# kerrm/vlite-fast

Measured on AMD Instinct MI355X. Metric: Msamp/s/antenna (dual-pol) and x real-time @128 MS/s; % HBM roofline, higher is better.
Workload: dtype f32

## Files before the change

### include/pb_hip.h

```cpp
#ifndef PB_HIP_H
#define PB_HIP_H

#include <stddef.h>
#include <stdint.h>

#ifdef __cplusplus
extern "C" {
#endif

#define PB_NFFT 12500
#define PB_NCHAN 6251
#define PB_NSCRUNCH 8
#define PB_NKURTO 500
#define PB_CHANMIN 2155
#define PB_CHANMAX 6250
#define PB_NCHANOUT 4096
#define PB_BLK_PER_FFT 25
#define PB_VDIF_FRAME 5032
#define PB_VDIF_DATA 5000
#define PB_FRAMES_PER_SEC 25600

#define PB_OK 0
#define PB_EINVAL (-22)
#define PB_ENOMEM (-12)
// ... 72 lines not shown
                         size_t nsamp_per_pol);
int pb_submit_vdif(pb_handle *h, int ant, int seg0, const uint8_t *block, size_t nbytes);
int pb_submit_vdif_at(pb_handle *h, int ant, int seg0, const uint8_t *block, size_t nbytes,
                      int64_t second, int64_t frame0);
int pb_input_dev(pb_handle *h, int ant, void **dptr, size_t *nbytes);

int pb_process(pb_handle *h, int nseg, int inject_now);

int pb_set_frb_params(pb_handle *h, float dm, float width_rows, float amp);

int pb_fetch(pb_handle *h, int ant, int seg0, int nseg, uint8_t *raw_codes, uint8_t *kur_codes,
             float *weights, float *ave_raw, float *ave_kur);
int pb_select_set(pb_handle *h, int set);
int pb_fetch_ptr(pb_handle *h, int ant, int stream, const uint8_t **codes);
int pb_output_dev(pb_handle *h, int ant, int stream, void **codes, void **ave);

int pb_coadd_local(pb_handle *h, int nseg, float *d_sum, int accumulate);
int pb_coadd_local_codes(pb_handle *h, int nseg, float *d_sum, int accumulate);
#define PB_COADD_MAX_LEAVES 32
int pb_coadd_tree_order(int n, int32_t *order);
int pb_coadd_local_tree(pb_handle *h, int nseg, const int32_t *ant_order, int n, float *d_dst);
int pb_coadd_tree(pb_handle *h, const float *const *d_leaves, int n, float *d_dst, size_t nfloat);
int pb_coadd_digitise(pb_handle *h, const float *d_sum, size_t nfloat, int nant_total, uint8_t *d_codes);
int pb_coadd_publish(pb_handle *h, const uint8_t *d_codes, size_t nbytes);
int pb_set_coadd_target(pb_handle *h, float *d_sum);
int pb_coadd_release(pb_handle *h);
int pb_set_coadd_stream(pb_handle *h, void *stream);
int pb_coadd_finish(pb_handle *h, int nseg, const float *d_sum, int nant_total,
                    uint8_t *codes_host);
int pb_coadd_fetch_ptr(pb_handle *h, int age, const uint8_t **codes);

int pb_profile(pb_handle *h, int enable);
int pb_get_timers(pb_handle *h, pb_timers *out, int reset);
int pb_debug_fetch(pb_handle *h, int what, int ant, int seg, void *dst, size_t nbytes);

int pb_debug_dag_check(pb_handle *h, float kur_lo, float kur_hi, uint64_t *nchecked, uint64_t *nmismatch,
                       float *bands4);

int pb_channelize_f32(pb_handle *h, const float *x, int nrows, int taps, float *out);

typedef struct pb_search pb_search;
int pb_search_create(int device, int nchan, int max_samples, float fch1_mhz, float foff_mhz, float tsamp_s,
                     float dm_min, float dm_max, float dm_step, int boxcar_max, const int *zap_ranges,
                     int nzap, pb_search **out);
int pb_search_create_list(int device, int nchan, int max_samples, float fch1_mhz, float foff_mhz, float tsamp_s,
                          const float *dm_list, int ndm, int boxcar_max, const int *zap_ranges, int nzap,
                          pb_search **out);
void pb_search_destroy(pb_search *s);
const char *pb_search_last_error(const pb_search *s);
int pb_search_info(const pb_search *s, int *ndm, int *nbox, int *max_delay);
int pb_search_run(pb_search *s, const void *codes, int codes_on_device, int nsamp, int nbit, float *snr,
                  uint8_t *width_log2, uint32_t *series, float *stats, int *tout);
int pb_search_set_baseline(pb_search *s, int window_samples);
int pb_search_peaks(pb_search *s, const void *codes, int codes_on_device, int nsamp, int nbit, float threshold,
                    int32_t *peaks, int max_out, int *npeaks, int *tout);
int pb_search_timers(const pb_search *s, float *ms6);

int pb_search_set_rfi(pb_search *s, int narrow, int broad, float tol, int rfi_boxcar_max);
int pb_search_rfi_info(const pb_search *s, uint64_t *n_narrow, int *n_broad_samples, float *ms);
int pb_search_fetch_clean(pb_search *s, uint8_t *xt, size_t nbytes);

int pb_search_set_cutouts(pb_search *s, int nsub, int nt, int ndmrow, int max_cands);
int pb_search_cutouts(pb_search *s, const int32_t *cands3, int n, uint32_t *ft, uint32_t *ft_hits, uint32_t *dt,
                      uint32_t *dt_hits);
int pb_search_cutout_timers(const pb_search *s, float *ms2);

int pb_search_set_refine(pb_search *s, int nstep, int half_window, int wmax, int max_cands);
int pb_search_refine(pb_search *s, const int32_t *req_i2, const float *req_f2, int n, int32_t *status, double *sn_dm,
                     int32_t *kbest, double *opt_sn, int32_t *opt_loc, uint32_t *series);
int pb_search_refine_timers(const pb_search *s, float *ms2);

int pb_search_set_pol(pb_search *s, int off_len, int guard, int nrm, double rm_lo, double rm_step, int max_cands);
int pb_search_pol(pb_search *s, const int32_t *req3, int n, int32_t *on, int32_t *non, int32_t *off, int32_t *noff, double *F,
                  int32_t *kbest, double *summary);
int pb_search_pol_cutouts(pb_search *s, const int32_t *cands3, int n, uint32_t *pft, uint32_t *pft_hits);
int pb_search_pol_fetch(pb_search *s, int which, uint8_t *out, size_t nbytes);
int pb_search_pol_timers(const pb_search *s, float *ms3);

#define PB_GIANT_WORDS 8
int pb_search_set_giants(pb_search *s, int sep_time, int sep_dm, int sep_filter, int max_giants);
int pb_search_giants(pb_search *s, float thresh, int t_lo, int t_hi, int32_t *cands, int max_out, int *ncands, int *ngiants,
                     int *overflow);
int pb_search_giant_list(pb_search *s, int32_t *out, int max_out, int *n);
int pb_search_set_planes(pb_search *s, const float *snr, const uint8_t *width_log2, int tout);
int pb_search_giant_timers(const pb_search *s, float *ms3, int *nsweeps);

int pb_search_set_gulp(pb_search *s, int keep_max);
int pb_search_push_f32(pb_search *s, const float *plane, int plane_on_device, int nsamp, float scale, int *fill);
int pb_search_push(pb_search *s, const void *codes, int codes_on_device, int nsamp, int nbit, int *fill);
int pb_search_gulp_peaks(pb_search *s, float threshold, int32_t *peaks, int max_out, int *npeaks, int *tout);
int pb_search_gulp_run(pb_search *s, float *snr, uint8_t *width_log2, uint32_t *series, float *stats, int *tout);
int pb_search_gulp_advance(pb_search *s, int keep);
int pb_search_gulp_fetch(pb_search *s, uint8_t *xt, size_t nbytes, int *fill);
int pb_search_gulp_timers(const pb_search *s, float *ms3);

void *pb_host_alloc(size_t nbytes);
void pb_host_free(void *p);

const char *pb_version(void);

#ifdef __cplusplus
}
#endif
#endif
```

### vlite-fast_amd/csrc/search_internal.h

```cpp
#pragma once
#include <hip/hip_runtime.h>

#include <cmath>
#include <cstdint>
#include <cstring>
#include <initializer_list>
#include <string>
#include <vector>

#include "pb_hip.h"

#define SEARCH_LOCAL __attribute__((visibility("hidden")))

struct pb_search {
    int device = 0, nchan = 0, max_samples = 0, ndm = 0, nbox = 0;
    float fch1 = 0.f, foff = 0.f, tsamp = 0.f;
    double dm_last = 0, ftop = 0;
    int max_delay = 0;
    uint8_t *d_codes = nullptr, *d_xt = nullptr;
    int32_t *d_delay = nullptr;
    int32_t *d_chans = nullptr;
    int nact = 0;
    uint32_t *d_D = nullptr;
    float *d_stats = nullptr;
    float *d_snr = nullptr;
    uint8_t *d_wid = nullptr;
    uint64_t *d_P = nullptr;
    int32_t *d_peaks = nullptr;
    int max_peaks = 1 << 20;
    int baseline = 0;
    int last_tout = 0, last_nsamp = 0;
    int plane_tout = 0;
    float ms[6] = {};
    hipEvent_t ev[7] = {};
    size_t tpitch = 0;
    hipStream_t stream = nullptr;
    std::string err;
    size_t ppitch() const { return tpitch + 8; }

    struct {
        int narrow = 0, broad = 0, nbox = 5;
        float tol = 5.0f;
        int ran = 0;
        int32_t *d_zdelay = nullptr;
        uint8_t *d_med = nullptr;
        uint32_t *d_z = nullptr;
        uint64_t *d_zP = nullptr;
        float *d_zstats = nullptr, *d_zsnr = nullptr;
        uint8_t *d_zwid = nullptr;
        int32_t *d_tlist = nullptr;
        unsigned long long *d_rcnt = nullptr;
        hipEvent_t ev[1] = {};
        uint64_t n_narrow = 0;
        int n_broad = 0;
        float ms = 0.f;
    } rfi;
    struct {
        int nsub = 0, nt = 0, ndmrow = 0, max = 0;
        int32_t *d_req = nullptr;
        int32_t *d_sub = nullptr;
        uint32_t *d_out = nullptr;
        uint32_t *h_out = nullptr;
        hipEvent_t ev[3] = {};
        float ms[2] = {};
    } cut;
    struct {
        int nstep = 0, H = 0, wmax = 0, max = 0;
        double *d_g = nullptr;
        int32_t *d_reqi = nullptr;
        float *d_reqf = nullptr;
        int32_t *d_out = nullptr;
        int32_t *h_out = nullptr;
        hipEvent_t ev[3] = {};
        float ms[2] = {};
    } rf;
    struct {
        int sep_time = 0, sep_dm = 0, sep_filter = 0, max = 0;
        int last = 0;
        int sweeps = 0;
        int32_t *d_cnt = nullptr, *d_row = nullptr;
        int32_t *d_giants = nullptr;
        int32_t *d_lab = nullptr;
        unsigned long long *d_best = nullptr;
        int32_t *d_acc = nullptr;
        int32_t *d_tile = nullptr;
        int32_t *d_out = nullptr;
        int32_t *h_out = nullptr;
        hipEvent_t ev[4] = {};
        float ms[3] = {};
    } gi;
    struct {
        int keep_max = 0;
// ... 32 lines not shown
extern SEARCH_LOCAL std::string g_search_err;

static inline int search_fail(pb_search *s, const char *fn, const std::string &what)
{
    (s ? s->err : g_search_err) = std::string(fn) + ": " + what;
    return PB_EINVAL;
}

#define SCHK(s, call)                                                         \
    do {                                                                      \
        hipError_t e_ = (call);                                               \
        if (e_ != hipSuccess) {                                               \
            (s)->err = std::string(#call) + ": " + hipGetErrorString(e_);     \
            return PB_EHIP;                                                   \
        }                                                                     \
    } while (0)

static inline int search_enter(pb_search *s, const char *fn, bool on, const char *off_msg, bool ready, const char *idle_msg)
{
    if (!s) return search_fail(nullptr, fn, "no search handle");
    if (!on) return search_fail(s, fn, off_msg);
    if (!ready) return search_fail(s, fn, idle_msg);
    return PB_OK;
}

static inline float search_ms(hipEvent_t a, hipEvent_t b)
{
    float ms = 0.f;
    return hipEventElapsedTime(&ms, a, b) == hipSuccess ? ms : 0.f;
}

static inline int search_get_ms(const pb_search *s, const float *ms, int n, float *out)
{
    if (!s || !out) return PB_EINVAL;
    for (int i = 0; i < n; ++i) out[i] = ms[i];
    return PB_OK;
}

static inline void search_release(std::initializer_list<void *> dev, void *host, hipEvent_t *ev, int nev)
{
    for (void *p : dev)
        if (p) (void)hipFree(p);
    if (host) (void)hipHostFree(host);
    for (int i = 0; i < nev; ++i)
        if (ev[i]) (void)hipEventDestroy(ev[i]);
}

SEARCH_LOCAL void search_rfi_free(pb_search *s);
SEARCH_LOCAL void search_cutouts_free(pb_search *s);
SEARCH_LOCAL void search_refine_free(pb_search *s);
SEARCH_LOCAL void search_giants_free(pb_search *s);
SEARCH_LOCAL void search_gulp_free(pb_search *s);
SEARCH_LOCAL void search_pol_free(pb_search *s);

SEARCH_LOCAL int search_pol_transpose(pb_search *s, const uint8_t *codes, int nsamp);
SEARCH_LOCAL void search_cutout_ft_launch(pb_search *s, const uint8_t *plane, int n, uint32_t *ft, uint32_t *fth);

SEARCH_LOCAL int search_block(pb_search *s, int nsamp, float thresh, bool want_peaks, bool cleaned);
SEARCH_LOCAL int search_run_out(pb_search *s, float *snr, uint8_t *width_log2, uint32_t *series, float *stats, int *tout_out);
SEARCH_LOCAL int search_peaks_out(pb_search *s, int32_t *peaks, int max_out, int *npeaks, int *tout_out);
```

### vlite-fast_amd/csrc/search_run.hip

```cpp
#include "search_internal.h"
#include "search_dev.h"

std::string g_search_err;

__global__ __launch_bounds__(256) void k_transpose_codes(const uint8_t *__restrict__ codes, uint8_t *__restrict__ xt,
                                                         int T, int nchan, int nbit, size_t tpitch)
{
    __shared__ uint8_t tile[64][65];
    const int t0 = blockIdx.x * 64, c0 = blockIdx.y * 64;
    const int per = 8 / nbit, maskv = (1 << nbit) - 1;
    for (int i = threadIdx.x; i < 64 * 64; i += 256) {
        const int tt = i / 64, cc = i % 64;
        const int t = t0 + tt, c = c0 + cc;
        uint8_t v = 0;
        if (t < T && c < nchan) {
            const size_t n = (size_t)t * nchan + c;
            v = (codes[n / per] >> (nbit * (n % per))) & maskv;
        }
        tile[tt][cc] = v;
    }
    __syncthreads();
    for (int i = threadIdx.x; i < 64 * 64; i += 256) {
        const int cc = i / 64, tt = i % 64;
        const int t = t0 + tt, c = c0 + cc;
// ... 410 lines not shown
    s->tsamp = tsamp_s;
    s->ndm = (int)dms.size();
    while ((1 << s->nbox) <= boxcar_max) s->nbox++;
    s->dm_last = dms.back();
    std::vector<int32_t> chans;
    for (int c = 0; c < nchan; ++c) {
        bool zap = false;
        for (int z = 0; z < nzap; ++z)
            if (c >= zap_ranges[2 * z] && c < zap_ranges[2 * z + 1]) zap = true;
        if (!zap) chans.push_back(c);
    }
    s->nact = (int)chans.size();
    if (s->nact == 0) {
        g_search_err = "pb_search_create: every channel is zapped";
        delete s;
        return PB_EINVAL;
    }
    std::vector<int32_t> delay((size_t)s->ndm * s->nact);
    const double ftop = foff_mhz < 0 ? fch1_mhz : fch1_mhz + (nchan - 1) * foff_mhz;
    s->ftop = ftop;
    int maxd = 0;
    for (int i = 0; i < s->ndm; ++i) {
        const double dm = dms[i];
        for (int k = 0; k < s->nact; ++k) {
            const double f = (double)fch1_mhz + (double)chans[k] * (double)foff_mhz;
            const int32_t di = delay_samples(dm, delay_chan_term(f, ftop), (double)tsamp_s);
            delay[(size_t)i * s->nact + k] = di;
            if (di > maxd) maxd = di;
        }
    }
    s->max_delay = maxd;
    s->tpitch = ((size_t)max_samples + 63) / 64 * 64;
    hipError_t e = hipSetDevice(device);
    if (e == hipSuccess) e = hipStreamCreateWithFlags(&s->stream, hipStreamNonBlocking);
    if (e == hipSuccess) e = hipMalloc((void **)&s->d_codes, (size_t)max_samples * nchan);
    if (e == hipSuccess) e = hipMalloc((void **)&s->d_xt, s->tpitch * nchan + 64);
    if (e == hipSuccess) e = hipMemset(s->d_xt, 0, s->tpitch * nchan + 64);
    if (e == hipSuccess) e = hipMalloc((void **)&s->d_delay, delay.size() * sizeof(int32_t));
    if (e == hipSuccess) e = hipMalloc((void **)&s->d_chans, chans.size() * sizeof(int32_t));
    if (e == hipSuccess) e = hipMemcpy(s->d_chans, chans.data(), chans.size() * sizeof(int32_t), hipMemcpyHostToDevice);
    if (e == hipSuccess) e = hipMalloc((void **)&s->d_D, (size_t)s->ndm * s->tpitch * sizeof(uint32_t));
    if (e == hipSuccess) e = hipMalloc((void **)&s->d_stats, (size_t)s->ndm * 2 * sizeof(float));
    if (e == hipSuccess) e = hipMalloc((void **)&s->d_snr, (size_t)s->ndm * s->tpitch * sizeof(float));
    if (e == hipSuccess) e = hipMalloc((void **)&s->d_wid, (size_t)s->ndm * s->tpitch);
    if (e == hipSuccess) e = hipMalloc((void **)&s->d_P, (size_t)s->ndm * s->ppitch() * sizeof(uint64_t));
    if (e == hipSuccess) e = hipMalloc((void **)&s->d_peaks, (size_t)(1 + 4 * s->max_peaks) * sizeof(int32_t));
    for (int i = 0; i < 7 && e == hipSuccess; ++i) e = hipEventCreate(&s->ev[i]);
    if (e == hipSuccess) e = hipMemcpy(s->d_delay, delay.data(), delay.size() * sizeof(int32_t), hipMemcpyHostToDevice);
    if (e != hipSuccess) {
        g_search_err = std::string("pb_search_create: ") + hipGetErrorString(e);
        pb_search_destroy(s);
        return PB_EHIP;
    }
    *out = s;
    return PB_OK;
}

void search_rfi_free(pb_search *s)
{
    search_release({s->rfi.d_zdelay, s->rfi.d_med, s->rfi.d_z, s->rfi.d_zP, s->rfi.d_zstats, s->rfi.d_zsnr, s->rfi.d_zwid,
                    s->rfi.d_tlist, s->rfi.d_rcnt}, nullptr, s->rfi.ev, 1);
    s->rfi = {};
}

extern "C" void pb_search_destroy(pb_search *s)
{
    if (!s) return;
    (void)hipSetDevice(s->device);
    if (s->stream) (void)hipStreamSynchronize(s->stream);
    search_rfi_free(s);
    search_cutouts_free(s);
    search_refine_free(s);
    search_giants_free(s);
    search_gulp_free(s);
    search_pol_free(s);
    search_release({s->d_codes, s->d_xt, s->d_delay, s->d_D, s->d_stats, s->d_snr, s->d_wid, s->d_P, s->d_peaks, s->d_chans},
                   nullptr, s->ev, 7);
    if (s->stream) (void)hipStreamDestroy(s->stream);
    delete s;
}

extern "C" int pb_search_info(const pb_search *s, int *ndm, int *nbox, int *max_delay)
{
    if (!s) return PB_EINVAL;
    if (ndm) *ndm = s->ndm;
    if (nbox) *nbox = s->nbox;
    if (max_delay) *max_delay = s->max_delay;
    return PB_OK;
}

extern "C" int pb_search_set_baseline(pb_search *s, int window_samples)
{
    if (!s || window_samples < 0) return PB_EINVAL;
    s->baseline = window_samples;
    return PB_OK;
}

extern "C" int pb_search_set_rfi(pb_search *s, int narrow, int broad, float tol, int rfi_boxcar_max)
{
    const char *fn = "pb_search_set_rfi";
    if (!(tol > 0) || !std::isfinite(tol)) return search_fail(s, fn, "tol must be > 0 and finite");
    if (rfi_boxcar_max < 1 || rfi_boxcar_max > 64 || (rfi_boxcar_max & (rfi_boxcar_max - 1)))
        return search_fail(s, fn, "rfi_boxcar_max must be a power of two in 1..64");
    if (!s) return search_fail(s, fn, "no search handle");
    if ((narrow || broad) && !s->rfi.d_rcnt) {
        const size_t tp = s->tpitch;
        SCHK(s, hipSetDevice(s->device));
        SCHK(s, hipMalloc((void **)&s->rfi.d_zdelay, (size_t)s->nact * sizeof(int32_t)));
        SCHK(s, hipMemset(s->rfi.d_zdelay, 0, (size_t)s->nact * sizeof(int32_t)));
        SCHK(s, hipMalloc((void **)&s->rfi.d_med, (size_t)s->nact));
        SCHK(s, hipMalloc((void **)&s->rfi.d_z, tp * sizeof(uint32_t)));
        SCHK(s, hipMalloc((void **)&s->rfi.d_zP, s->ppitch() * sizeof(uint64_t)));
        SCHK(s, hipMalloc((void **)&s->rfi.d_zstats, 2 * sizeof(float)));
        SCHK(s, hipMalloc((void **)&s->rfi.d_zsnr, tp * sizeof(float)));
        SCHK(s, hipMalloc((void **)&s->rfi.d_zwid, tp));
        SCHK(s, hipMalloc((void **)&s->rfi.d_tlist, tp * sizeof(int32_t)));
        SCHK(s, hipEventCreate(&s->rfi.ev[0]));
        SCHK(s, hipMalloc((void **)&s->rfi.d_rcnt, 2 * sizeof(unsigned long long)));
    }
    s->rfi.narrow = narrow != 0;
    s->rfi.broad = broad != 0;
    s->rfi.tol = tol;
    s->rfi.nbox = 0;
    while ((1 << s->rfi.nbox) <= rfi_boxcar_max) s->rfi.nbox++;
    return PB_OK;
}

static int search_clean(pb_search *s, int nsamp)
{
    const size_t ppitch = s->ppitch();
    SCHK(s, hipMemsetAsync(s->rfi.d_rcnt, 0, 2 * sizeof(unsigned long long), s->stream));
    k_rfi_narrow<<<s->nact, 256, 0, s->stream>>>(s->d_xt, s->d_chans, s->rfi.d_med, nsamp, s->tpitch, s->rfi.tol,
                                                 s->rfi.narrow, s->rfi.d_rcnt);
    if (s->rfi.broad) {
        dim3 gz((nsamp + DDM_TILE - 1) / DDM_TILE, 1);
        k_dedisperse<<<gz, 256, 0, s->stream>>>(s->d_xt, s->d_chans, s->rfi.d_zdelay, s->rfi.d_z, s->nact, 1, nsamp, s->tpitch,
                                                s->tpitch);
        k_prefix<<<1, 256, 0, s->stream>>>(s->rfi.d_z, s->rfi.d_zP, nsamp, s->tpitch, ppitch);
        k_series_stats<<<1, 256, 0, s->stream>>>(s->rfi.d_z, s->rfi.d_zP, s->rfi.d_zstats, nsamp, s->baseline, s->tpitch, ppitch);
        dim3 gb((nsamp + 255) / 256, 1);
        k_boxcar<<<gb, 256, 0, s->stream>>>(s->rfi.d_zP, s->rfi.d_zstats, s->rfi.d_zsnr, s->rfi.d_zwid, nsamp, s->rfi.nbox, s->baseline,
                                            s->tpitch, ppitch, 0.f, nullptr, 0);
        k_rfi_broad_list<<<gb, 256, 0, s->stream>>>(s->rfi.d_zsnr, s->rfi.d_zwid, nsamp, s->rfi.tol, 1 << (s->rfi.nbox - 1),
                                                    s->rfi.d_tlist, s->rfi.d_rcnt + 1);
        k_rfi_broad_mask<<<(s->nact + 3) / 4, 256, 0, s->stream>>>(s->d_xt, s->d_chans, s->rfi.d_med, s->rfi.d_tlist,
                                                                   s->rfi.d_rcnt + 1, s->nact, s->tpitch);
    }
    SCHK(s, hipEventRecord(s->rfi.ev[0], s->stream));
    return PB_OK;
}

int search_block(pb_search *s, int nsamp, float thresh, bool want_peaks, bool cleaned)
{
    const int tout = nsamp - s->max_delay;
    s->rfi.ran = s->rfi.narrow || s->rfi.broad;
    if (s->rfi.ran && cleaned) {
        SCHK(s, hipEventRecord(s->rfi.ev[0], s->stream));
    } else if (s->rfi.ran) {
        const int rc = search_clean(s, nsamp);
        if (rc) return rc;
    }
    dim3 gd((tout + 255) / 256, s->ndm);
    dim3 gdd((tout + DDM_TILE - 1) / DDM_TILE, (s->ndm + DDM_DB - 1) / DDM_DB);
    k_dedisperse<<<gdd, 256, 0, s->stream>>>(s->d_xt, s->d_chans, s->d_delay, s->d_D, s->nact, s->ndm, tout, s->tpitch, s->tpitch);
    SCHK(s, hipEventRecord(s->ev[3], s->stream));
    const size_t ppitch = s->ppitch();
    k_prefix<<<s->ndm, 256, 0, s->stream>>>(s->d_D, s->d_P, tout, s->tpitch, ppitch);
    k_series_stats<<<s->ndm, 256, 0, s->stream>>>(s->d_D, s->d_P, s->d_stats, tout, s->baseline, s->tpitch, ppitch);
    SCHK(s, hipEventRecord(s->ev[4], s->stream));
    if (want_peaks) SCHK(s, hipMemsetAsync(s->d_peaks, 0, sizeof(int32_t), s->stream));
    k_boxcar<<<gd, 256, 0, s->stream>>>(s->d_P, s->d_stats, s->d_snr, s->d_wid, tout, s->nbox, s->baseline, s->tpitch,
                                        ppitch, thresh, want_peaks ? s->d_peaks : nullptr, s->max_peaks);
    SCHK(s, hipEventRecord(s->ev[5], s->stream));
    SCHK(s, hipGetLastError());
    s->last_tout = tout;
    s->last_nsamp = nsamp;
    s->plane_tout = tout;
    return PB_OK;
}

static int search_run(pb_search *s, const void *codes, int codes_on_device, int nsamp, int nbit, float thresh,
                      bool want_peaks)
{
    if (!s || !codes) return PB_EINVAL;
    if (nsamp > s->max_samples || !(nbit == 8 || nbit == 4 || nbit == 2))
        return search_fail(s, "pb_search_run", "block too long or bad nbit");
    const int tout = nsamp - s->max_delay;
    if (tout < 64) return search_fail(s, "pb_search_run", "block shorter than the largest dispersion delay");
    SCHK(s, hipSetDevice(s->device));
    const bool pol = s->pol.max > 0;
    if (pol && nbit != 8) return search_fail(s, "pb_search_run", "with polarisation on the block must be 8-bit");
    const size_t nbytes = (size_t)nsamp * s->nchan * nbit / 8 * (pol ? 4 : 1);
    const uint8_t *d_codes = (const uint8_t *)codes;
    s->gp.fill = 0;
    s->gp.cleaned = 0;
    s->gp.tail_n = 0;
    SCHK(s, hipEventRecord(s->ev[0], s->stream));
    if (!codes_on_device) {
        uint8_t *stage = pol ? s->pol.d_codes : s->d_codes;
        SCHK(s, hipMemcpyAsync(stage, codes, nbytes, hipMemcpyHostToDevice, s->stream));
        d_codes = stage;
    }
    SCHK(s, hipEventRecord(s->ev[1], s->stream));
    if (pol) {
        const int rc = search_pol_transpose(s, d_codes, nsamp);
        if (rc) return rc;
    } else {
        dim3 gt((nsamp + 63) / 64, (s->nchan + 63) / 64);
        k_transpose_codes<<<gt, 256, 0, s->stream>>>(d_codes, s->d_xt, nsamp, s->nchan, nbit, s->tpitch);
    }
    SCHK(s, hipEventRecord(s->ev[2], s->stream));
    return search_block(s, nsamp, thresh, want_peaks, false);
}

static int search_times(pb_search *s)
{
    for (int i = 0; i < 6; ++i) s->ms[i] = search_ms((i == 2 && s->rfi.ran) ? s->rfi.ev[0] : s->ev[i], s->ev[i + 1]);
// ... 86 lines not shown
```

### vlite-fast_amd/libpb.py

```python
import ctypes as C
import os

import numpy as np

_HERE = os.path.dirname(os.path.abspath(__file__))
LIB_PATH = os.environ.get("PB_LIBPATH") or os.path.join(_HERE, "csrc", "libpb_hip.so")

NFFT = 12500
NCHAN = 6251
NSCRUNCH = 8
NKURTO = 500
CHANMIN = 2155
CHANMAX = 6250
NCHANOUT = 4096
VLITE_RATE = 128000000
FFT_LDS = 0
FFT_HIPFFT = 1

STAGES = ("kurtosis", "channelize", "fft", "inject", "detect", "deframe", "coadd", "h2d")
DBG_POW, DBG_KUR, DBG_DAG, DBG_FLAGS, DBG_ROWWEIGHT, DBG_POW_FB, DBG_KUR_FB, DBG_DAG_FB = range(8)


class PbError(RuntimeError):
    pass


class PbConfig(C.Structure):
    _fields_ = [("struct_size", C.c_uint32), ("device", C.c_int32), ("nant", C.c_int32),
                ("nbit", C.c_int32), ("npol", C.c_int32), ("rfi_mode", C.c_int32),
                ("taps", C.c_int32), ("fft_backend", C.c_int32), ("rows_per_seg", C.c_int32),
                ("max_seg", C.c_int32), ("inject_frb", C.c_int32), ("keep_ave", C.c_int32),
                ("debug_keep", C.c_int32), ("nsets", C.c_int32), ("coherence", C.c_int32)]


class PbSizes(C.Structure):
    _fields_ = [("seg_samples_per_pol", C.c_uint64), ("input_bytes_per_seg", C.c_uint64),
                ("code_bytes_per_seg", C.c_uint64), ("ave_floats_per_seg", C.c_uint64),
                ("rows_per_seg", C.c_uint64), ("blocks_per_seg_pol", C.c_uint64),
                ("device_bytes", C.c_uint64)]


class PbTimers(C.Structure):
    _fields_ = [("ms", C.c_double * 8), ("launches", C.c_uint64 * 8)]


EXPORTS = ["pb_config_default", "pb_create", "pb_destroy", "pb_last_error", "pb_query",
           "pb_set_stream", "pb_sync", "pb_reset_bandpass", "pb_reset_history", "pb_get_bandpass", "pb_set_bandpass",
           "pb_submit_planar", "pb_submit_planar_dev", "pb_submit_vdif", "pb_submit_vdif_at", "pb_input_dev", "pb_process", "pb_set_frb_params", "pb_select_set", "pb_fetch", "pb_fetch_ptr",
           "pb_output_dev", "pb_coadd_local", "pb_coadd_local_codes", "pb_coadd_local_tree", "pb_coadd_tree", "pb_coadd_tree_order", "pb_coadd_digitise", "pb_coadd_publish", "pb_set_coadd_target", "pb_coadd_release", "pb_set_coadd_stream", "pb_coadd_finish", "pb_coadd_fetch_ptr", "pb_profile", "pb_get_timers", "pb_host_alloc", "pb_host_free",
           "pb_debug_fetch", "pb_debug_dag_check", "pb_channelize_f32", "pb_version", "pb_search_create", "pb_search_create_list", "pb_search_destroy",
           "pb_search_last_error", "pb_search_info", "pb_search_run", "pb_search_set_baseline", "pb_search_peaks",
           "pb_search_timers", "pb_search_set_rfi", "pb_search_rfi_info", "pb_search_fetch_clean", "pb_search_set_cutouts",
           "pb_search_cutouts", "pb_search_cutout_timers", "pb_search_set_refine", "pb_search_refine",
           "pb_search_refine_timers", "pb_search_set_giants", "pb_search_giants", "pb_search_giant_list",
           "pb_search_set_planes", "pb_search_giant_timers", "pb_search_set_gulp", "pb_search_push", "pb_search_push_f32", "pb_search_gulp_peaks",
           "pb_search_gulp_run", "pb_search_gulp_advance", "pb_search_gulp_fetch", "pb_search_gulp_timers", "pb_search_set_pol",
           "pb_search_pol", "pb_search_pol_cutouts", "pb_search_pol_fetch", "pb_search_pol_timers"]

_lib = None


def load():
    global _lib
    if _lib is not None:
        return _lib
    if not os.path.exists(LIB_PATH):
        raise PbError("%s not found: build it with `make -C vlite-fast_amd/csrc`; "
                      "there is no CPU fallback" % LIB_PATH)
    if os.environ.get("PB_NO_TORCH_PRELOAD") != "1":
        try:
            import torch
        except Exception:
            pass
    L = C.CDLL(LIB_PATH)
    vp, u8p, fp = C.c_void_p, C.POINTER(C.c_uint8), C.POINTER(C.c_float)
    L.pb_config_default.argtypes = [C.POINTER(PbConfig)]
    L.pb_config_default.restype = None
    L.pb_create.argtypes = [C.POINTER(PbConfig), C.POINTER(vp)]
    L.pb_destroy.argtypes = [vp]
    L.pb_destroy.restype = None
    L.pb_last_error.argtypes = [vp]
    L.pb_last_error.restype = C.c_char_p
    L.pb_query.argtypes = [vp, C.POINTER(PbSizes)]
    L.pb_set_stream.argtypes = [vp, vp]
    L.pb_sync.argtypes = [vp]
    L.pb_reset_bandpass.argtypes = [vp, C.c_int]
    L.pb_reset_history.argtypes = [vp, C.c_int]
    L.pb_get_bandpass.argtypes = [vp, C.c_int, fp, fp]
    L.pb_set_bandpass.argtypes = [vp, C.c_int, fp, fp]
    L.pb_submit_planar.argtypes = [vp, C.c_int, C.c_int, u8p, u8p, C.c_size_t]
    L.pb_submit_planar_dev.argtypes = [vp, C.c_int, C.c_int, vp, vp, C.c_size_t]
    L.pb_submit_vdif.argtypes = [vp, C.c_int, C.c_int, u8p, C.c_size_t]
    L.pb_submit_vdif_at.argtypes = [vp, C.c_int, C.c_int, u8p, C.c_size_t, C.c_int64, C.c_int64]
    L.pb_input_dev.argtypes = [vp, C.c_int, C.POINTER(vp), C.POINTER(C.c_size_t)]
    L.pb_process.argtypes = [vp, C.c_int, C.c_int]
    L.pb_fetch.argtypes = [vp, C.c_int, C.c_int, C.c_int, u8p, u8p, fp, fp, fp]
    L.pb_set_frb_params.argtypes = [vp, C.c_float, C.c_float, C.c_float]
    L.pb_select_set.argtypes = [vp, C.c_int]
    L.pb_fetch_ptr.argtypes = [vp, C.c_int, C.c_int, C.POINTER(u8p)]
    L.pb_output_dev.argtypes = [vp, C.c_int, C.c_int, C.POINTER(vp), C.POINTER(vp)]
    L.pb_coadd_local.argtypes = [vp, C.c_int, vp, C.c_int]
    L.pb_coadd_local_codes.argtypes = [vp, C.c_int, vp, C.c_int]
    L.pb_coadd_local_tree.argtypes = [vp, C.c_int, C.POINTER(C.c_int32), C.c_int, vp]
    L.pb_coadd_tree.argtypes = [vp, C.POINTER(vp), C.c_int, vp, C.c_size_t]
    L.pb_coadd_tree_order.argtypes = [C.c_int, C.POINTER(C.c_int32)]
    L.pb_coadd_digitise.argtypes = [vp, vp, C.c_size_t, C.c_int, vp]
    L.pb_coadd_publish.argtypes = [vp, vp, C.c_size_t]
    L.pb_set_coadd_target.argtypes = [vp, vp]
    L.pb_coadd_release.argtypes = [vp]
    L.pb_set_coadd_stream.argtypes = [vp, vp]
    L.pb_coadd_finish.argtypes = [vp, C.c_int, vp, C.c_int, u8p]
    L.pb_coadd_fetch_ptr.argtypes = [vp, C.c_int, C.POINTER(u8p)]
    L.pb_profile.argtypes = [vp, C.c_int]
    L.pb_get_timers.argtypes = [vp, C.POINTER(PbTimers), C.c_int]
    L.pb_debug_fetch.argtypes = [vp, C.c_int, C.c_int, C.c_int, vp, C.c_size_t]
    L.pb_channelize_f32.argtypes = [vp, fp, C.c_int, C.c_int, fp]
    L.pb_debug_dag_check.argtypes = [vp, C.c_float, C.c_float, C.POINTER(C.c_uint64), C.POINTER(C.c_uint64), fp]
    L.pb_version.restype = C.c_char_p
    L.pb_host_alloc.argtypes = [C.c_size_t]
    L.pb_host_alloc.restype = vp
    L.pb_host_free.argtypes = [vp]
    L.pb_host_free.restype = None
    ip = C.POINTER(C.c_int)
    L.pb_search_create.argtypes = [C.c_int, C.c_int, C.c_int, C.c_float, C.c_float, C.c_float, C.c_float, C.c_float,
                                   C.c_float, C.c_int, ip, C.c_int, C.POINTER(vp)]
    L.pb_search_create_list.argtypes = [C.c_int, C.c_int, C.c_int, C.c_float, C.c_float, C.c_float, fp, C.c_int, C.c_int,
                                        ip, C.c_int, C.POINTER(vp)]
    L.pb_search_destroy.argtypes = [vp]
    L.pb_search_destroy.restype = None
    L.pb_search_last_error.argtypes = [vp]
    L.pb_search_last_error.restype = C.c_char_p
    L.pb_search_info.argtypes = [vp, ip, ip, ip]
    L.pb_search_run.argtypes = [vp, vp, C.c_int, C.c_int, C.c_int, fp, u8p, C.POINTER(C.c_uint32), fp, ip]
    L.pb_search_set_baseline.argtypes = [vp, C.c_int]
    L.pb_search_peaks.argtypes = [vp, vp, C.c_int, C.c_int, C.c_int, C.c_float, C.POINTER(C.c_int32), C.c_int, ip, ip]
    L.pb_search_timers.argtypes = [vp, fp]
    L.pb_search_set_rfi.argtypes = [vp, C.c_int, C.c_int, C.c_float, C.c_int]
    L.pb_search_rfi_info.argtypes = [vp, C.POINTER(C.c_uint64), ip, fp]
    L.pb_search_fetch_clean.argtypes = [vp, u8p, C.c_size_t]
    u32p = C.POINTER(C.c_uint32)
    L.pb_search_set_cutouts.argtypes = [vp, C.c_int, C.c_int, C.c_int, C.c_int]
    L.pb_search_cutouts.argtypes = [vp, C.POINTER(C.c_int32), C.c_int, u32p, u32p, u32p, u32p]
    L.pb_search_cutout_timers.argtypes = [vp, fp]
    i32p, f64p = C.POINTER(C.c_int32), C.POINTER(C.c_double)
    L.pb_search_set_refine.argtypes = [vp, C.c_int, C.c_int, C.c_int, C.c_int]
    L.pb_search_refine.argtypes = [vp, i32p, fp, C.c_int, i32p, f64p, i32p, f64p, i32p, u32p]
    L.pb_search_refine_timers.argtypes = [vp, fp]
    L.pb_search_set_giants.argtypes = [vp, C.c_int, C.c_int, C.c_int, C.c_int]
    L.pb_search_giants.argtypes = [vp, C.c_float, C.c_int, C.c_int, i32p, C.c_int, ip, ip, ip]
    L.pb_search_giant_list.argtypes = [vp, i32p, C.c_int, ip]
    L.pb_search_set_planes.argtypes = [vp, fp, u8p, C.c_int]
    L.pb_search_giant_timers.argtypes = [vp, fp, ip]
    L.pb_search_set_gulp.argtypes = [vp, C.c_int]
    L.pb_search_push.argtypes = [vp, vp, C.c_int, C.c_int, C.c_int, ip]
    L.pb_search_push_f32.argtypes = [vp, vp, C.c_int, C.c_int, C.c_float, ip]
    L.pb_search_gulp_peaks.argtypes = [vp, C.c_float, i32p, C.c_int, ip, ip]
    L.pb_search_gulp_run.argtypes = [vp, fp, u8p, u32p, fp, ip]
    L.pb_search_gulp_advance.argtypes = [vp, C.c_int]
    L.pb_search_gulp_fetch.argtypes = [vp, u8p, C.c_size_t, ip]
    L.pb_search_gulp_timers.argtypes = [vp, fp]
    L.pb_search_set_pol.argtypes = [vp, C.c_int, C.c_int, C.c_int, C.c_double, C.c_double, C.c_int]
    L.pb_search_pol.argtypes = [vp, i32p, C.c_int, i32p, i32p, i32p, i32p, f64p, i32p, f64p]
    L.pb_search_pol_cutouts.argtypes = [vp, i32p, C.c_int, u32p, u32p]
    L.pb_search_pol_fetch.argtypes = [vp, C.c_int, u8p, C.c_size_t]
    L.pb_search_pol_timers.argtypes = [vp, fp]
    for n in EXPORTS:
        f = getattr(L, n)
        if f.restype is C.c_int or n in ("pb_create", "pb_query", "pb_sync"):
            f.restype = C.c_int
    _lib = L
    return L


def _u8(a):
    return a.ctypes.data_as(C.POINTER(C.c_uint8)) if a is not None else None


def _f32(a):
    return a.ctypes.data_as(C.POINTER(C.c_float)) if a is not None else None


class PbHandle(object):

    def __init__(self, device=0, nant=1, nbit=8, npol=1, rfi_mode=2, taps=1, fft_backend=FFT_LDS,
                 rows_per_seg=1024, max_seg=10, inject_frb=False, keep_ave=False, debug_keep=False,
                 nsets=1, coherence=False):
        L = load()
# ... 205 lines not shown
```

### vlite-fast_amd/search.py

```python
import ctypes as C
import importlib

import numpy as np

_pkg = __package__ or "vlite-fast_amd"

HEIMDALL_DM = (2.0, 1000.0)
HEIMDALL_BOXCAR_MAX = 64
HEIMDALL_GULP = 30720
HEIMDALL_ZAP = ((0, 190), (3900, 4096))
FCH1 = 384 + (2155 - 0.5) * (-64. / 6251)
FOFF = -64. / 6251
TSAMP = 12500.0 / 128e6 * 8


def dedisp_dm_list(dm_start, dm_end, tsamp, fch1, foff, nchan, tol=1.25, pulse_width_us=40.0):
    dt = tsamp * 1e6
    f = (fch1 + (nchan / 2 - 0.5) * foff) * 1e-3
    tol2 = tol * tol
    a = 8.3 * abs(foff) / (f * f * f)
    a2 = a * a
    b2 = a2 * (nchan * nchan / 16.0)
    c = (dt * dt + pulse_width_us * pulse_width_us) * (tol2 - 1.0)
    dms = [float(dm_start)]
    while dms[-1] < dm_end:
        prev = dms[-1]
        k = c + tol2 * a2 * prev * prev
        dms.append((b2 * prev + np.sqrt(-a2 * b2 * prev * prev + (a2 + b2) * k)) / (a2 + b2))
    return np.asarray(dms, np.float32)


class Searcher(object):
    def __init__(self, device=0, nchan=4096, max_samples=HEIMDALL_GULP, fch1=FCH1, foff=FOFF, tsamp=TSAMP,
                 dm_min=HEIMDALL_DM[0], dm_max=HEIMDALL_DM[1], dm_step=2.0, boxcar_max=HEIMDALL_BOXCAR_MAX,
                 zap=HEIMDALL_ZAP, dm_list=None):
        lp = importlib.import_module(_pkg + ".libpb")
        self._lp = lp
        self._L = lp.load()
        zr = (C.c_int * (2 * len(zap)))(*[v for pair in zap for v in pair])
        self._s = C.c_void_p()
        if dm_list is not None:
            dl = np.ascontiguousarray(dm_list, np.float32)
            rc = self._L.pb_search_create_list(device, nchan, max_samples, fch1, foff, tsamp,
                                               dl.ctypes.data_as(C.POINTER(C.c_float)), dl.size, boxcar_max, zr, len(zap),
                                               C.byref(self._s))
        else:
            rc = self._L.pb_search_create(device, nchan, max_samples, fch1, foff, tsamp, dm_min, dm_max, dm_step,
                                          boxcar_max, zr, len(zap), C.byref(self._s))
        self._check(rc, "pb_search_create", handle=False)
        ndm, nbox, md = C.c_int(), C.c_int(), C.c_int()
        self._L.pb_search_info(self._s, C.byref(ndm), C.byref(nbox), C.byref(md))
        self.ndm, self.nbox, self.max_delay = ndm.value, nbox.value, md.value
        self.nchan, self.tsamp = nchan, tsamp
        self.max_samples = max_samples
        self.fch1, self.foff = fch1, foff
        self._cut = None
        self._ref = None
        self._gi = None
        self._pol = None
        self.dms = dm_min + dm_step * np.arange(self.ndm) if dm_list is None else np.asarray(dm_list, np.float64)
        self._nsamp = 0
        self._tout = 0

    def _check(self, rc, name, exc=None, handle=True):
        if rc != 0:
            err = self._L.pb_search_last_error(self._s if handle else None).decode()
            raise exc(err) if exc else self._lp.PbError("%s failed (%d): %s" % (name, rc, err))

    def close(self):
        if getattr(self, "_s", None):
            self._L.pb_search_destroy(self._s)
            self._s = None

    def __enter__(self):
        return self

    def __exit__(self, *a):
        self.close()

    def __del__(self):
        try:
            self.close()
        except Exception:
            pass

    def set_baseline(self, window_samples):
        rc = self._L.pb_search_set_baseline(self._s, int(window_samples))
        if rc != 0:
            raise ValueError("baseline window must be >= 0")

    def set_rfi(self, narrow=True, broad=True, tol=5.0, boxcar_max=16):
        rc = self._L.pb_search_set_rfi(self._s, int(bool(narrow)), int(bool(broad)), float(tol), int(boxcar_max))
        self._check(rc, None, ValueError)

    def rfi_info(self):
        n, b, ms = C.c_uint64(), C.c_int(), C.c_float()
        self._L.pb_search_rfi_info(self._s, C.byref(n), C.byref(b), C.byref(ms))
        return dict(n_narrow=int(n.value), n_broad_samples=int(b.value), ms=float(ms.value))

    def fetch_clean(self):
        out = np.empty((self.nchan, self._nsamp), np.uint8)
        rc = self._L.pb_search_fetch_clean(self._s, out.ctypes.data_as(C.POINTER(C.c_uint8)), out.nbytes)
        self._check(rc, "pb_search_fetch_clean")
        return out

    def set_cutouts(self, nsub=64, nt=256, ndmrow=64, max_cands=32):
        rc = self._L.pb_search_set_cutouts(self._s, int(nsub), int(nt), int(ndmrow), int(max_cands))
        self._check(rc, None, ValueError)
        self._cut = (int(nsub), int(nt), int(ndmrow), int(max_cands)) if max_cands else None

    def cutouts(self, dmi, t, tscr):
        if self._cut is None:
            raise self._lp.PbError("cutouts are not switched on: call set_cutouts() first")
        nsub, nt, nrow, _ = self._cut
        req = np.stack(np.broadcast_arrays(np.atleast_1d(dmi), np.atleast_1d(t), np.atleast_1d(tscr)), axis=1)
        req = np.ascontiguousarray(req, np.int32)
        n = req.shape[0]
        out = dict(ft=np.zeros((n, nsub, nt), np.uint32), ft_hits=np.zeros((n, nsub, nt), np.uint32),
                   dt=np.zeros((n, nrow, nt), np.uint32), dt_hits=np.zeros((n, nrow, nt), np.uint32))
        u32p = C.POINTER(C.c_uint32)
        rc = self._L.pb_search_cutouts(self._s, req.ctypes.data_as(C.POINTER(C.c_int32)), n,
                                       *[out[k].ctypes.data_as(u32p) for k in ("ft", "ft_hits", "dt", "dt_hits")])
        self._check(rc, "pb_search_cutouts")
        rows = req[:, :1].astype(np.int64) - nrow // 2 + np.arange(nrow)[None, :]
        ok = (rows >= 0) & (rows < self.ndm)
        out["dm_rows"] = np.where(ok, np.asarray(self.dms, np.float64)[np.clip(rows, 0, self.ndm - 1)], np.nan)
        per = self.nchan // nsub
        out["sub_freqs"] = self.fch1 + self.foff * (np.arange(nsub) * per + (per - 1) / 2.0)
        return out

    def cutout_timers(self):
        t = (C.c_float * 2)()
        self._L.pb_search_cutout_timers(self._s, t)
        return dict(kernels=float(t[0]), with_copy=float(t[1]))

    def set_pol(self, off_len=64, guard=8, rm=(-2000.0, 2.0, 2001), max_cands=32):
        lo, step, nrm = float(rm[0]), float(rm[1]), int(rm[2])
# ... 895 lines not shown
```

Before: 213,800.

## Add LDS-staged dedispersion kernel for DM blocks with small delay spread

New measurement: 212,900. About the same (-0.4%).

```diff
diff --git a/include/pb_hip.h b/include/pb_hip.h
--- a/include/pb_hip.h
+++ b/include/pb_hip.h
@@ -148,6 +148,11 @@
 int pb_search_run(pb_search *s, const void *codes, int codes_on_device, int nsamp, int nbit, float *snr,
                   uint8_t *width_log2, uint32_t *series, float *stats, int *tout);
 int pb_search_set_baseline(pb_search *s, int window_samples);
+#define PB_DEDISP_AUTO 0
+#define PB_DEDISP_TILE 1
+#define PB_DEDISP_LDS 2
+int pb_search_set_dedisp(pb_search *s, int mode);
+int pb_search_dedisp_info(const pb_search *s, int *staged_rows, int *tiled_rows, int *window_bytes);
 int pb_search_peaks(pb_search *s, const void *codes, int codes_on_device, int nsamp, int nbit, float threshold,
                     int32_t *peaks, int max_out, int *npeaks, int *tout);
 int pb_search_timers(const pb_search *s, float *ms6);
diff --git a/vlite-fast_amd/csrc/search_dedisp.hip b/vlite-fast_amd/csrc/search_dedisp.hip
--- /dev/null
+++ b/vlite-fast_amd/csrc/search_dedisp.hip
@@ -0,0 +1,189 @@
+#include "search_internal.h"
+#include "search_dev.h"
+
+typedef uint32_t dl_u32x2 __attribute__((ext_vector_type(2), aligned(4)));
+typedef uint32_t dl_lds2 __attribute__((ext_vector_type(2)));
+typedef const __attribute__((address_space(3))) uint8_t *dl_ldsp;
+typedef uint32_t dl_u32x8 __attribute__((ext_vector_type(8)));
+
+#define DL_AHEAD 3
+#define DL_IT_MAX 4
+static_assert(DL_IT_MAX * 64 * 8 >= dl_win_bytes(DL_SPREAD_CAP), "a wave stages a whole window in DL_IT_MAX sweeps");
+static_assert(DL_CG == 8 && DL_NB == 16 && DL_TT == 512, "4 waves x 2 channels staged, 4 waves x 4 DMs, 64 lanes x 8 samples");
+
+template <int IT>
+__global__ __launch_bounds__(256, 4) void k_dedisperse_lds(const uint8_t *__restrict__ xt, const int32_t *__restrict__ chans,
+                                                        const int32_t *__restrict__ base, const int32_t *__restrict__ blks,
+                                                        const dl_u32x8 *__restrict__ code, uint32_t *__restrict__ D, int nact,
+                                                        int ndm, int tout, int nsamp, size_t tpitch, size_t dpitch, int win)
+{
+    extern __shared__ __attribute__((aligned(16))) uint8_t dl_lds[];
+    const int wave = __builtin_amdgcn_readfirstlane(threadIdx.x >> 6), lane = threadIdx.x & 63;
+    const int blk = blks[blockIdx.y];
+    const int t0 = blockIdx.x * DL_TT, t = t0 + 8 * lane;
+    const int32_t *bs = base + (size_t)blk * nact;
+    const int nrow = min(DL_NB, ndm - blk * DL_NB) - 4 * wave;
+    const int ng = (nact + DL_CG - 1) / DL_CG;
+    const dl_u32x8 *cd[4];
+    uint32_t lo[4][2], hi[4][2], acc[4][8];
+#pragma unroll
+    for (int j = 0; j < 4; ++j) {
+        cd[j] = code + (size_t)(blockIdx.y * DL_NB + 4 * wave + j) * (2 * ng);
+        lo[j][0] = lo[j][1] = hi[j][0] = hi[j][1] = 0u;
+#pragma unroll
+        for (int i = 0; i < 8; ++i) acc[j][i] = 0u;
+    }
+    const int cp = 2 * win + 8;
+    const int bufsz = DL_CG * cp;
+
+    dl_u32x2 pre[2][IT];
+    int sc_chan[2], sc_base[2];
+    auto fetch = [&](int c0) {
+#pragma unroll
+        for (int u = 0; u < 2; ++u) {
+            const int c = min(c0 + wave + 4 * u, nact - 1);
+            sc_chan[u] = chans[c];
+            sc_base[u] = bs[c];
+        }
+    };
+    auto load = [&](int c0) {
+#pragma unroll
+        for (int u = 0; u < 2; ++u) {
+            const bool live = c0 + wave + 4 * u < nact;
+            const uint8_t *row = xt + (size_t)sc_chan[u] * tpitch;
+            const int s = dl_win_start(t0, sc_base[u]);
+#pragma unroll
+            for (int i = 0; i < IT; ++i) {
+                const int p = lane + 64 * i, x = s + 8 * p;
+                dl_u32x2 v = {0u, 0u};
+                if (live && 8 * p < win && dl_pair_loaded(x, nsamp)) v = *(const dl_u32x2 *)(row + x);
+                pre[u][i] = v;
+            }
+        }
+    };
+    auto store = [&](uint8_t *b) {
+#pragma unroll
+        for (int u = 0; u < 2; ++u) {
+            uint8_t *A = b + (wave + 4 * u) * cp, *B = A + win + 8;
+#pragma unroll
+            for (int i = 0; i < IT; ++i) {
+                const int p = lane + 64 * i;
+                if (8 * p < win) {
+                    *(uint2 *)(A + 8 * p) = make_uint2(pre[u][i].x, pre[u][i].y);
+                    *(uint32_t *)(B + 8 * p - 4) = pre[u][i].x;
+                    *(uint32_t *)(B + 8 * p) = pre[u][i].y;
+                }
+            }
+        }
+    };
+    auto flush = [&]() {
+#pragma unroll
+        for (int j = 0; j < 4; ++j) {
+#pragma unroll
+            for (int w = 0; w < 2; ++w) {
+                acc[j][4 * w + 0] += lo[j][w] & 0xffffu;
+                acc[j][4 * w + 1] += hi[j][w] & 0xffffu;
+                acc[j][4 * w + 2] += lo[j][w] >> 16;
+                acc[j][4 * w + 3] += hi[j][w] >> 16;
+                lo[j][w] = hi[j][w] = 0u;
+            }
+        }
+    };
+
+    fetch(0);
+    load(0);
+    fetch(DL_CG);
+    store(dl_lds);
+    __syncthreads();
+    int since = 0;
+    for (int g = 0; g < ng; ++g) {
+        if (g + 1 < ng) load((g + 1) * DL_CG);
+        fetch((g + 2) * DL_CG);
+        const dl_ldsp b = (dl_ldsp)(dl_lds + (g & 1) * bufsz + 8 * lane);
+#pragma unroll
+        for (int jj = 0; jj < 4; jj += 2) {
+            const dl_u32x8 ca[2] = {cd[jj][2 * g], cd[jj + 1][2 * g]}, cb[2] = {cd[jj][2 * g + 1], cd[jj + 1][2 * g + 1]};
+            dl_lds2 v[DL_AHEAD + 1][2];
+            auto entry = [&](int i, int e) {
+                const int k = 2 * (i >> 2) + (i & 1), j = (i >> 1) & 1;
+                return k < 4 ? ca[j][2 * k + e] : cb[j][2 * (k - 4) + e];
+            };
+            auto read = [&](int i) {
+                const dl_ldsp q = b + entry(i, 0);
+                v[i % (DL_AHEAD + 1)][0] = *(const volatile __attribute__((address_space(3))) dl_lds2 *)q;
+                v[i % (DL_AHEAD + 1)][1] = *(const volatile __attribute__((address_space(3))) dl_lds2 *)(q + 8);
+            };
+#pragma unroll
+            for (int i = 0; i < DL_AHEAD; ++i) read(i);
+#pragma unroll
+            for (int i = 0; i < 2 * DL_CG; ++i) {
+                if (i + DL_AHEAD < 2 * DL_CG) read(i + DL_AHEAD);
+                const int j = jj + ((i >> 1) & 1);
+                const dl_lds2 v0 = v[i % (DL_AHEAD + 1)][0], v1 = v[i % (DL_AHEAD + 1)][1];
+                const uint32_t sl = entry(i, 1), sh = sl + 0x00010001u;
+                lo[j][0] += __builtin_amdgcn_perm(v0.y, v0.x, sl);
+                hi[j][0] += __builtin_amdgcn_perm(v0.y, v0.x, sh);
+                lo[j][1] += __builtin_amdgcn_perm(v1.x, v0.y, sl);
+                hi[j][1] += __builtin_amdgcn_perm(v1.x, v0.y, sh);
+            }
+            __builtin_amdgcn_sched_barrier(0);
+        }
+        since += DL_CG;
+        if (since >= GATHER_FLUSH) {
+            flush();
+            since = 0;
+        }
+        if (g + 1 < ng) store(dl_lds + ((g + 1) & 1) * bufsz);
+        __syncthreads();
+    }
+    flush();
+    if (t >= tout) return;
+#pragma unroll
+    for (int j = 0; j < 4; ++j) {
+        if (j >= nrow) break;
+        uint32_t *out = D + (size_t)(blk * DL_NB + 4 * wave + j) * dpitch + t;
+#pragma unroll
+        for (int i = 0; i < 8; i += 4) {
+            if (t + i + 4 <= tout) {
+                *(uint4 *)(out + i) = make_uint4(acc[j][i], acc[j][i + 1], acc[j][i + 2], acc[j][i + 3]);
+            } else {
+                for (int q = 0; q < 4; ++q)
+                    if (t + i + q < tout) out[i + q] = acc[j][i + q];
+            }
+        }
+    }
+}
+
+int search_dedisp_plan(pb_search *s, const int32_t *delay, int mode)
+{
+    const dl_plan p = dl_make_plan(delay, s->ndm, s->nact, mode);
+    search_dedisp_free(s);
+    s->dd.mode = mode;
+    s->dd.win = p.win;
+    s->dd.nstaged = (int)p.staged.size();
+    s->dd.rest = p.rest;
+    if (!s->dd.nstaged) return PB_OK;
+    SCHK(s, hipMalloc((void **)&s->dd.d_base, p.base.size() * sizeof(int32_t)));
+    SCHK(s, hipMalloc((void **)&s->dd.d_blks, p.staged.size() * sizeof(int32_t)));
+    SCHK(s, hipMalloc((void **)&s->dd.d_code, p.code.size() * sizeof(uint32_t)));
+    SCHK(s, hipMemcpy(s->dd.d_code, p.code.data(), p.code.size() * sizeof(uint32_t), hipMemcpyHostToDevice));
+    SCHK(s, hipMemcpy(s->dd.d_base, p.base.data(), p.base.size() * sizeof(int32_t), hipMemcpyHostToDevice));
+    SCHK(s, hipMemcpy(s->dd.d_blks, p.staged.data(), p.staged.size() * sizeof(int32_t), hipMemcpyHostToDevice));
+    return PB_OK;
+}
+
+void search_dedisp_free(pb_search *s)
+{
+    search_release({s->dd.d_base, s->dd.d_blks, s->dd.d_code}, nullptr, nullptr, 0);
+    s->dd = {};
+}
+
+void search_dedisp_lds_launch(pb_search *s, int nsamp, int tout)
+{
+    const dim3 g((tout + DL_TT - 1) / DL_TT, s->dd.nstaged);
+    const size_t lds = (size_t)2 * DL_CG * (2 * s->dd.win + 8);
+    const int it = (s->dd.win / 8 + 63) / 64;
+    auto k = it <= 2 ? k_dedisperse_lds<2> : it == 3 ? k_dedisperse_lds<3> : k_dedisperse_lds<DL_IT_MAX>;
+    k<<<g, 256, lds, s->stream>>>(s->d_xt, s->d_chans, s->dd.d_base, s->dd.d_blks, (const dl_u32x8 *)s->dd.d_code, s->d_D, s->nact, s->ndm,
+                                  tout, nsamp, s->tpitch, s->tpitch, s->dd.win);
+}
diff --git a/vlite-fast_amd/csrc/search_internal.h b/vlite-fast_amd/csrc/search_internal.h
--- a/vlite-fast_amd/csrc/search_internal.h
+++ b/vlite-fast_amd/csrc/search_internal.h
@@ -9,6 +9,7 @@
 #include <vector>
 
 #include "pb_hip.h"
+#include "search_plan.h"
 
 #define SEARCH_LOCAL __attribute__((visibility("hidden")))
 
@@ -38,6 +39,14 @@
     std::string err;
     size_t ppitch() const { return tpitch + 8; }
 
+    struct {
+        int mode = DL_MODE_AUTO, nstaged = 0, win = 0;
+        int32_t *d_base = nullptr;
+        int32_t *d_blks = nullptr;
+        uint32_t *d_code = nullptr;
+        std::vector<int32_t> rest;
+    } dd;
+    std::vector<int32_t> h_delay;
     struct {
         int narrow = 0, broad = 0, nbox = 5;
         float tol = 5.0f;
@@ -176,6 +185,10 @@
 SEARCH_LOCAL void search_giants_free(pb_search *s);
 SEARCH_LOCAL void search_gulp_free(pb_search *s);
 SEARCH_LOCAL void search_pol_free(pb_search *s);
+SEARCH_LOCAL void search_dedisp_free(pb_search *s);
+
+SEARCH_LOCAL int search_dedisp_plan(pb_search *s, const int32_t *delay, int mode);
+SEARCH_LOCAL void search_dedisp_lds_launch(pb_search *s, int nsamp, int tout);
 
 SEARCH_LOCAL int search_pol_transpose(pb_search *s, const uint8_t *codes, int nsamp);
 SEARCH_LOCAL void search_cutout_ft_launch(pb_search *s, const uint8_t *plane, int n, uint32_t *ft, uint32_t *fth);
diff --git a/vlite-fast_amd/csrc/search_plan.h b/vlite-fast_amd/csrc/search_plan.h
--- /dev/null
+++ b/vlite-fast_amd/csrc/search_plan.h
@@ -0,0 +1,78 @@
+#pragma once
+#include <cstdint>
+#include <vector>
+
+#define DL_NB 16
+#define DL_TT 512
+#define DL_SPREAD_CAP 1024
+#define DL_CG 8
+
+enum { DL_MODE_AUTO = 0, DL_MODE_TILE = 1, DL_MODE_LDS = 2 };
+
+constexpr int dl_win_start(int t0, int base) { return (t0 + base) & ~3; }
+constexpr int dl_win_bytes(int spread) { return ((((spread + 3) & ~3) + 8 * 63 + 16) + 7) & ~7; }
+constexpr bool dl_pair_loaded(int x, int nsamp) { return x + 8 <= nsamp + 16; }
+
+constexpr uint32_t dl_read_off(int c, int r, int win) { return (uint32_t)((c % DL_CG) * (2 * win + 8) + (r & ~7) + ((r & 4) ? win + 8 : 0)); }
+constexpr uint32_t dl_read_sel(int r) { return 0x0c020c00u + (uint32_t)(r & 3) * 0x00010001u; }
+
+struct dl_plan {
+    int nblk = 0;
+    int win = 0;
+    std::vector<int32_t> base;
+    std::vector<int32_t> spread;
+    std::vector<int32_t> staged;
+    std::vector<int32_t> rest;
+    std::vector<uint32_t> code;
+};
+
+inline dl_plan dl_make_plan(const int32_t *delay, int ndm, int nact, int mode)
+{
+    dl_plan p;
+    p.nblk = (ndm + DL_NB - 1) / DL_NB;
+    p.base.assign((size_t)p.nblk * nact, 0);
+    p.spread.assign(p.nblk, 0);
+    int top = 0;
+    for (int b = 0; b < p.nblk; ++b) {
+        const int r0 = b * DL_NB, r1 = r0 + DL_NB < ndm ? r0 + DL_NB : ndm;
+        int sp = 0;
+        for (int c = 0; c < nact; ++c) {
+            int32_t lo = delay[(size_t)r0 * nact + c], hi = lo;
+            for (int r = r0 + 1; r < r1; ++r) {
+                const int32_t d = delay[(size_t)r * nact + c];
+                if (d < lo) lo = d;
+                if (d > hi) hi = d;
+            }
+            p.base[(size_t)b * nact + c] = lo;
+            if (hi - lo > sp) sp = hi - lo;
+        }
+        p.spread[b] = sp;
+        const bool stage = mode != DL_MODE_TILE && sp <= DL_SPREAD_CAP;
+        if (stage) {
+            p.staged.push_back(b);
+            if (sp > top) top = sp;
+        } else if (!p.rest.empty() && p.rest[p.rest.size() - 2] + p.rest.back() == r0) {
+            p.rest.back() += r1 - r0;
+        } else {
+            p.rest.push_back(r0);
+            p.rest.push_back(r1 - r0);
+        }
+    }
+    p.win = dl_win_bytes(top);
+    const size_t cpitch = (size_t)((nact + DL_CG - 1) / DL_CG * DL_CG);
+    p.code.resize(p.staged.size() * DL_NB * cpitch * 2);
+    for (size_t i = 0; i < p.staged.size(); ++i) {
+        const int b = p.staged[i];
+        for (int j = 0; j < DL_NB; ++j) {
+            const bool row = b * DL_NB + j < ndm;
+            const int32_t *d = delay + (size_t)(row ? b * DL_NB + j : 0) * nact;
+            uint32_t *q = p.code.data() + (i * DL_NB + j) * cpitch * 2;
+            for (int c = 0; c < (int)cpitch; ++c) {
+                const int r = row && c < nact ? d[c] - (p.base[(size_t)b * nact + c] & ~3) : 0;
+                q[2 * c] = dl_read_off(c, r, p.win);
+                q[2 * c + 1] = dl_read_sel(r);
+            }
+        }
+    }
+    return p;
+}
diff --git a/vlite-fast_amd/csrc/search_run.hip b/vlite-fast_amd/csrc/search_run.hip
--- a/vlite-fast_amd/csrc/search_run.hip
+++ b/vlite-fast_amd/csrc/search_run.hip
@@ -486,6 +486,12 @@
         pb_search_destroy(s);
         return PB_EHIP;
     }
+    s->h_delay = std::move(delay);
+    if (search_dedisp_plan(s, s->h_delay.data(), DL_MODE_AUTO) != PB_OK) {
+        g_search_err = "pb_search_create: " + s->err;
+        pb_search_destroy(s);
+        return PB_EHIP;
+    }
     *out = s;
     return PB_OK;
 }
@@ -508,6 +514,7 @@
     search_giants_free(s);
     search_gulp_free(s);
     search_pol_free(s);
+    search_dedisp_free(s);
     search_release({s->d_codes, s->d_xt, s->d_delay, s->d_D, s->d_stats, s->d_snr, s->d_wid, s->d_P, s->d_peaks, s->d_chans},
                    nullptr, s->ev, 7);
     if (s->stream) (void)hipStreamDestroy(s->stream);
@@ -527,6 +534,27 @@
 {
     if (!s || window_samples < 0) return PB_EINVAL;
     s->baseline = window_samples;
+    return PB_OK;
+}
+
+extern "C" int pb_search_set_dedisp(pb_search *s, int mode)
+{
+    if (!s) return search_fail(nullptr, "pb_search_set_dedisp", "no search handle");
+    if (mode != PB_DEDISP_AUTO && mode != PB_DEDISP_TILE && mode != PB_DEDISP_LDS)
+        return search_fail(s, "pb_search_set_dedisp", "mode must be 0 (auto), 1 (tile) or 2 (lds)");
+    SCHK(s, hipSetDevice(s->device));
+    SCHK(s, hipStreamSynchronize(s->stream));
+    return search_dedisp_plan(s, s->h_delay.data(), mode);
+}
+
+extern "C" int pb_search_dedisp_info(const pb_search *s, int *staged_rows, int *tiled_rows, int *window_bytes)
+{
+    if (!s) return PB_EINVAL;
+    int rest = 0;
+    for (size_t i = 1; i < s->dd.rest.size(); i += 2) rest += s->dd.rest[i];
+    if (staged_rows) *staged_rows = s->dd.nstaged ? s->ndm - rest : 0;
+    if (tiled_rows) *tiled_rows = s->dd.nstaged ? rest : s->ndm;
+    if (window_bytes) *window_bytes = s->dd.nstaged ? s->dd.win : 0;
     return PB_OK;
 }
 
@@ -596,7 +624,17 @@
     }
     dim3 gd((tout + 255) / 256, s->ndm);
     dim3 gdd((tout + DDM_TILE - 1) / DDM_TILE, (s->ndm + DDM_DB - 1) / DDM_DB);
-    k_dedisperse<<<gdd, 256, 0, s->stream>>>(s->d_xt, s->d_chans, s->d_delay, s->d_D, s->nact, s->ndm, tout, s->tpitch, s->tpitch);
+    if (!s->dd.nstaged) {
+        k_dedisperse<<<gdd, 256, 0, s->stream>>>(s->d_xt, s->d_chans, s->d_delay, s->d_D, s->nact, s->ndm, tout, s->tpitch, s->tpitch);
+    } else {
+        search_dedisp_lds_launch(s, nsamp, tout);
+        for (size_t i = 0; i + 1 < s->dd.rest.size(); i += 2) {
+            const int r0 = s->dd.rest[i], nr = s->dd.rest[i + 1];
+            const dim3 gr(gdd.x, (nr + DDM_DB - 1) / DDM_DB);
+            k_dedisperse<<<gr, 256, 0, s->stream>>>(s->d_xt, s->d_chans, s->d_delay + (size_t)r0 * s->nact,
+                                                    s->d_D + (size_t)r0 * s->tpitch, s->nact, nr, tout, s->tpitch, s->tpitch);
+        }
+    }
     SCHK(s, hipEventRecord(s->ev[3], s->stream));
     const size_t ppitch = s->ppitch();
     k_prefix<<<s->ndm, 256, 0, s->stream>>>(s->d_D, s->d_P, tout, s->tpitch, ppitch);
diff --git a/vlite-fast_amd/libpb.py b/vlite-fast_amd/libpb.py
--- a/vlite-fast_amd/libpb.py
+++ b/vlite-fast_amd/libpb.py
@@ -49,7 +49,7 @@
            "pb_submit_planar", "pb_submit_planar_dev", "pb_submit_vdif", "pb_submit_vdif_at", "pb_input_dev", "pb_process", "pb_set_frb_params", "pb_select_set", "pb_fetch", "pb_fetch_ptr",
            "pb_output_dev", "pb_coadd_local", "pb_coadd_local_codes", "pb_coadd_local_tree", "pb_coadd_tree", "pb_coadd_tree_order", "pb_coadd_digitise", "pb_coadd_publish", "pb_set_coadd_target", "pb_coadd_release", "pb_set_coadd_stream", "pb_coadd_finish", "pb_coadd_fetch_ptr", "pb_profile", "pb_get_timers", "pb_host_alloc", "pb_host_free",
            "pb_debug_fetch", "pb_debug_dag_check", "pb_channelize_f32", "pb_version", "pb_search_create", "pb_search_create_list", "pb_search_destroy",
-           "pb_search_last_error", "pb_search_info", "pb_search_run", "pb_search_set_baseline", "pb_search_peaks",
+           "pb_search_last_error", "pb_search_info", "pb_search_run", "pb_search_set_baseline", "pb_search_set_dedisp", "pb_search_dedisp_info", "pb_search_peaks",
            "pb_search_timers", "pb_search_set_rfi", "pb_search_rfi_info", "pb_search_fetch_clean", "pb_search_set_cutouts",
            "pb_search_cutouts", "pb_search_cutout_timers", "pb_search_set_refine", "pb_search_refine",
            "pb_search_refine_timers", "pb_search_set_giants", "pb_search_giants", "pb_search_giant_list",
@@ -133,6 +133,8 @@
     L.pb_search_info.argtypes = [vp, ip, ip, ip]
     L.pb_search_run.argtypes = [vp, vp, C.c_int, C.c_int, C.c_int, fp, u8p, C.POINTER(C.c_uint32), fp, ip]
     L.pb_search_set_baseline.argtypes = [vp, C.c_int]
+    L.pb_search_set_dedisp.argtypes = [vp, C.c_int]
+    L.pb_search_dedisp_info.argtypes = [vp, ip, ip, ip]
     L.pb_search_peaks.argtypes = [vp, vp, C.c_int, C.c_int, C.c_int, C.c_float, C.POINTER(C.c_int32), C.c_int, ip, ip]
     L.pb_search_timers.argtypes = [vp, fp]
     L.pb_search_set_rfi.argtypes = [vp, C.c_int, C.c_int, C.c_float, C.c_int]
diff --git a/vlite-fast_amd/search.py b/vlite-fast_amd/search.py
--- a/vlite-fast_amd/search.py
+++ b/vlite-fast_amd/search.py
@@ -1,5 +1,6 @@
 import ctypes as C
 import importlib
+import os
 
 import numpy as np
 
@@ -12,6 +13,7 @@
 FCH1 = 384 + (2155 - 0.5) * (-64. / 6251)
 FOFF = -64. / 6251
 TSAMP = 12500.0 / 128e6 * 8
+DEDISP_MODES = {"auto": 0, "tile": 1, "lds": 2}
 
 
 def dedisp_dm_list(dm_start, dm_end, tsamp, fch1, foff, nchan, tol=1.25, pulse_width_us=40.0):
@@ -48,6 +50,12 @@
             rc = self._L.pb_search_create(device, nchan, max_samples, fch1, foff, tsamp, dm_min, dm_max, dm_step,
                                           boxcar_max, zr, len(zap), C.byref(self._s))
         self._check(rc, "pb_search_create", handle=False)
+        mode = os.environ.get("PB_SEARCH_DEDISP", "auto")
+        if mode not in DEDISP_MODES:
+            self.close()
+            raise ValueError("PB_SEARCH_DEDISP must be one of auto, tile, lds")
+        if mode != "auto":
+            self._check(self._L.pb_search_set_dedisp(self._s, DEDISP_MODES[mode]), "pb_search_set_dedisp")
         ndm, nbox, md = C.c_int(), C.c_int(), C.c_int()
         self._L.pb_search_info(self._s, C.byref(ndm), C.byref(nbox), C.byref(md))
         self.ndm, self.nbox, self.max_delay = ndm.value, nbox.value, md.value
@@ -83,6 +91,11 @@
             self.close()
         except Exception:
             pass
+
+    def dedisp_info(self):
+        a, b, w = C.c_int(), C.c_int(), C.c_int()
+        self._L.pb_search_dedisp_info(self._s, C.byref(a), C.byref(b), C.byref(w))
+        return dict(staged=a.value, tiled=b.value, window_bytes=w.value)
 
     def set_baseline(self, window_samples):
         rc = self._L.pb_search_set_baseline(self._s, int(window_samples))
```
